# graph-embedding/node2vec

Hardware: AMD Instinct MI355X
Metric: walk-steps/sec + embedding-updates/sec on 100M-node synthetic; 1/2/4/8 GPU (higher is better)
Workload: dtype f64

## Files before the change

### node2vec_amd/csrc/n2v_walk_fast.hip

```cpp
#include "n2v_common.h"

namespace n2v {

__device__ __forceinline__ bool member_pivoted_lane(const int32_t *col, const int32_t *pivots,
                                                    int64_t first, int m, int32_t x) {
  const int64_t last = first + m;
  int64_t lo = first >> 5, hi = (last - 1) >> 5;
  while (lo < hi) {
    const int64_t mid = (lo + hi) >> 1;
    if (pivots[mid] < x)
      lo = mid + 1;
    else
      hi = mid;
  }
  int64_t a = max(first, lo << 5);
  const int64_t end = min(last, (lo << 5) + 32);
  int64_t b = end;
  while (a < b) {
    const int64_t mid = (a + b) >> 1;
    if (col[mid] < x)
      a = mid + 1;
    else
      b = mid;
  }
  return a < end && col[a] == x;
}

__global__ void pivots_build_kernel(const int32_t *__restrict__ col, int64_t n_edges,
                                    int32_t *__restrict__ pivots) {
  const int64_t n_blocks = (n_edges + 31) >> 5;
  for (int64_t j = (int64_t)blockIdx.x * blockDim.x + threadIdx.x; j < n_blocks;
       j += (int64_t)gridDim.x * blockDim.x)
    pivots[j] = col[min(32 * j + 31, n_edges - 1)];
}

__device__ __forceinline__ int lower_bound_lane(const int32_t *a, int m, int32_t x) {
  int lo = 0, hi = m;
  while (lo < hi) {
    const int mid = (lo + hi) >> 1;
    if (a[mid] < x)
      lo = mid + 1;
    else
      hi = mid;
  }
  return lo;
}

template <bool kUnit, bool kHops, bool kClassFirst, bool kSlots = false>
__global__ __launch_bounds__(256, 6) void walk_fast_kernel(
    n2v_graph g, const int32_t *__restrict__ start_ids, int64_t n_start, int32_t num_walks,
    int32_t walk_length, double p, double q, uint64_t seed, int32_t *__restrict__ walks_out,
    uint8_t *__restrict__ valid_out, uint32_t *__restrict__ status,
    unsigned long long *__restrict__ trials_out) {
  const int64_t total = n_start * (int64_t)num_walks;
  const int64_t n_lanes = (int64_t)gridDim.x * blockDim.x;
  const int L1 = walk_length + 1;
  const double inv_p = 1.0 / p, inv_q = 1.0 / q;
  const double b_lo = fmin(1.0, inv_q), b_hi = fmax(1.0, inv_q);
  const double beta_max = fmax(b_hi, inv_p);
  const bool biased = !(p == 1.0 && q == 1.0);
  const bool have_ec = kUnit && (kHops || g.edge_classes != nullptr);
  const bool have_w = have_ec && g.wedge_off != nullptr && g.wedge_pos != nullptr;
  const bool slots_tab = kSlots && have_w && g.wedge_wide != 1 && g.wedge_slots != nullptr;
  const bool inl_tab = kHops && (g.reserved2 & N2V_HOPS_INLINE_RPOS) != 0;
  int rpos_inl = -1;
  int64_t e_prev = 0;
  const bool fold_return = have_ec && inv_p > b_hi;
  const bool base_aligned = (reinterpret_cast<uintptr_t>(walks_out) & 63u) == 0;

  int64_t r = (int64_t)blockIdx.x * blockDim.x + threadIdx.x;
  bool live = false;
  int32_t s = -1, v = 0;
  int step = 0;
  uint32_t trial = 0;
  int64_t vb = 0, sb = 0, w0 = 0;
  int n = 0, m = 0;
  uint64_t h0 = 0, hstep = 0;
  unsigned long long trials = 0;
  double rho = -1.0;
  int shared = -1;
  int n_ret = 0;
  int cls = -1;
  double m_l1 = 0.0, m_l12 = 0.0, m_tot = 0.0;
  int c1 = 4, c3 = 1;
  double w1 = 0.0, d2 = 0.0, d3 = 0.0;
  if (kClassFirst) {
    double wc[3] = {inv_p, 1.0, inv_q};
    int bc[3] = {1, 2, 4};
    for (int a = 0; a < 2; ++a)
      for (int b = 0; b < 2 - a; ++b)
        if (wc[b] > wc[b + 1]) {
          const double tw = wc[b]; wc[b] = wc[b + 1]; wc[b + 1] = tw;
          const int tb = bc[b]; bc[b] = bc[b + 1]; bc[b + 1] = tb;
        }
    c1 = bc[0];
    c3 = bc[2];
    w1 = wc[0];
    d2 = wc[1] - wc[0];
    d3 = wc[2] - wc[1];
  }

  __shared__ int32_t path_tile[16][256];
  const int tid = threadIdx.x;
  int lo = 0;
  auto put = [&](int64_t a, int32_t x) { path_tile[(int)(a & 15)][tid] = x; };
  auto flush = [&](int64_t a) {
    const int k = (int)(a & 15);
    int32_t *sec = walks_out + (a & ~(int64_t)15);
    if (lo == 0 && k == 15 && base_aligned) {
#pragma unroll
      for (int u = 0; u < 4; ++u)
        reinterpret_cast<int4 *>(sec)[u] =
            make_int4(path_tile[4 * u][tid], path_tile[4 * u + 1][tid], path_tile[4 * u + 2][tid],
                      path_tile[4 * u + 3][tid]);
    } else {
      for (int kk = lo; kk <= k; ++kk) sec[kk] = path_tile[kk][tid];
    }
    lo = 0;
  };
  auto emit = [&](int pos, int32_t x) {
    const int64_t a = w0 + pos;
    put(a, x);
    if ((a & 15) == 15 || pos == walk_length) flush(a);
  };

  auto begin_walker = [&]() -> bool {
    while (r < total) {
      const int32_t start = start_ids[r / num_walks];
      const int32_t ordinal = (int32_t)(r % num_walks) + 1;
      w0 = r * (int64_t)L1;
      lo = (int)(w0 & 15);
      bool ok = true;
      if (start < 0 || (int64_t)start >= g.n_vertices) {
        atomicOr(status, N2V_ST_RANGE);
        ok = false;
      }
      if (ok) {
        vb = g.rowptr[start];
        n = (int)(g.rowptr[start + 1] - vb);
        ok = n > 0;
      }
      if (!ok || walk_length == 0) {
        emit(0, ok ? start : -1);
        for (int t = 1; t < L1; ++t) emit(t, -1);
        valid_out[r] = ok ? 1 : 0;
        r += n_lanes;
        continue;
      }
      s = -1;
      v = start;
      step = 0;
      trial = 0;
      rho = -1.0;
      shared = -1;
      cls = -1;
      emit(0, start);
      h0 = walker_stream(seed, (uint64_t)start * (uint64_t)num_walks + (uint64_t)(ordinal - 1));
      hstep = step_bits(h0, 0);
      return true;
    }
    return false;
  };

  live = begin_walker();
  while (__ballot(live) != 0ull) {
    if (!live) continue;
    const bool plain = s < 0 || !biased;
    const uint64_t bits = plain ? hstep : trial_bits(hstep, trial);
    const uint32_t u1 = (uint32_t)(bits >> 32), u2 = (uint32_t)bits;
    int pick = pick_index(u1, n);
    const bool w_wide = wedge_row_wide(g.wedge_wide, n);
    const bool have_slots = slots_tab && !w_wide;
    uint64_t wraw = 0;
    int4 ws_a = make_int4(0, 0, 0, 0), ws_b = make_int4(0, 0, 0, 0);
    if (kClassFirst && !plain) {
      if (cls < 0) {
        const double uc = (double)u2 * (1.0 / 4294967296.0) * m_tot;
        double ul = uc, wl = w1;
        cls = 7;
        if (!(uc < m_l1)) {
          if (uc < m_l12) {
            cls = 7 & ~c1;
            ul = uc - m_l1;
            wl = d2;
          } else {
            cls = c3;
            ul = uc - m_l12;
            wl = d3;
          }
        }
        if (!(cls & 4)) {
          const int cnt_r = (cls & 1) ? n_ret : 0, cnt_m = (cls & 2) ? shared : 0;
          int kk = (int)(ul / wl);
          kk = kk < cnt_r + cnt_m ? kk : cnt_r + cnt_m - 1;
          kk = kk < 0 ? 0 : kk;
          if (rpos_inl >= 0 && cnt_m == 0) {
            pick = rpos_inl + kk;
          } else if (have_slots) {
            const int4 *slot = reinterpret_cast<const int4 *>(g.wedge_slots + e_prev * 16);
            ws_a = slot[0];
            ws_b = slot[1];
            pick = kk < cnt_r ? (int)((uint32_t)ws_a.x & 0xffffu) + kk
                              : slot_entry(ws_a, ws_b, shared, kk - cnt_r,
                                           reinterpret_cast<const uint16_t *>(g.wedge_pos));
          } else {
            wraw = g.wedge_off[e_prev];
            if (kk < cnt_r) {
              pick = (int)(wraw >> N2V_WEDGE_RPOS_SHIFT) + kk;
            } else {
              const int64_t off = (int64_t)(wraw & N2V_WEDGE_OFF_MASK) + (kk - cnt_r);
              pick = w_wide ? (int)reinterpret_cast<const uint32_t *>(g.wedge_pos)[off]
                            : (int)reinterpret_cast<const uint16_t *>(g.wedge_pos)[off];
            }
          }
// ... 74 lines not shown
      }
    }
    if (!accept) {
      ++trial;
      continue;
    }
    emit(step + 1, x);
    e_prev = e;
    s = v;
    sb = vb;
    m = n;
    v = x;
    ++step;
    trial = 0;
    cls = -1;
    const bool finished = step == walk_length;
    bool dropped = false;
    if (!finished) {
      if (kHops) {
        vb = hop_row(h);
        n = hop_deg(h);
      } else {
        vb = g.rowptr[v];
        n = (int)(g.rowptr[v + 1] - vb);
      }
      dropped = n == 0;
      hstep = step_bits(h0, (uint32_t)step);
      rho = -1.0;
      shared = -1;
      if (kClassFirst) {
        uint32_t ec = kHops ? h.classes : g.edge_classes[e];
        rpos_inl = -1;
        if (inl_tab && ec != 0xffffffffu && (ec & N2V_EC_INLINE) != 0u) {
          rpos_inl = (int)(ec & N2V_EC_SHARED_MASK);
          ec = ((ec >> N2V_EC_RETURN_SHIFT) & 0x7fu) << N2V_EC_RETURN_SHIFT;
        }
        n_ret = (int)(ec >> N2V_EC_RETURN_SHIFT);
        shared = q != 1.0 ? (int)(ec & N2V_EC_SHARED_MASK) : 0;
        const int n_oth = n - n_ret - shared;
        const int n_c1 = c1 == 1 ? n_ret : (c1 == 2 ? shared : n_oth);
        const int n_c3 = c3 == 1 ? n_ret : (c3 == 2 ? shared : n_oth);
        m_l1 = (double)n * w1;
        m_l12 = m_l1 + (double)(n - n_c1) * d2;
        m_tot = m_l12 + (double)n_c3 * d3;
      } else if (have_ec && biased && !dropped) {
        uint32_t ec = kHops ? h.classes : g.edge_classes[e];
        if (inl_tab && ec != 0xffffffffu && (ec & N2V_EC_INLINE) != 0u)
          ec = ((ec >> N2V_EC_RETURN_SHIFT) & 0x7fu) << N2V_EC_RETURN_SHIFT;
        const uint32_t fR = ec >> N2V_EC_RETURN_SHIFT, fM = ec & N2V_EC_SHARED_MASK;
        if (fM != N2V_EC_SHARED_MASK) shared = (int)fM;
        if (fold_return && fR != N2V_EC_RETURN_SAT) {
          const double wr = (double)fR * inv_p;
          rho = wr / (wr + (double)n * b_hi);
        }
      }
    }
    if (finished || dropped) {
      if (dropped)
        for (int t = step + 1; t < L1; ++t) emit(t, -1);
      valid_out[r] = finished ? 1 : 0;
      r += n_lanes;
      live = begin_walker();
    }
  }
  if (trials_out && trials) atomicAdd(trials_out, trials);
}

}

extern "C" int n2v_walk_fast_launch(const n2v_graph *g, const int32_t *start_ids,
                                    int64_t n_start, int32_t num_walks, int32_t walk_length,
                                    double p, double q, uint64_t seed, int32_t *walks_out,
                                    uint8_t *valid_out, uint32_t *status, void *stream) {
  const int64_t total = n_start * (int64_t)num_walks;
  if (total == 0) return N2V_OK;
  const bool unit = g->w == nullptr && g->w64 == nullptr;
  if (!unit && !g->slots) return N2V_EINVAL;
  const int threads = 256;
  int64_t blocks = (total + threads - 1) / threads;
  const bool hops = unit && g->hops != nullptr;
  const bool cf = unit && (hops || g->edge_classes) && g->wedge_off && g->wedge_pos &&
                  !(p == 1.0 && q == 1.0);
  const bool slots = cf && hops && q < 1.0 && g->wedge_slots && g->wedge_wide != 1;
  const void *fn = slots  ? (const void *)n2v::walk_fast_kernel<true, true, true, true>
                   : cf   ? (hops ? (const void *)n2v::walk_fast_kernel<true, true, true>
                                  : (const void *)n2v::walk_fast_kernel<true, false, true>)
                   : hops ? (const void *)n2v::walk_fast_kernel<true, true, false>
                   : unit ? (const void *)n2v::walk_fast_kernel<true, false, false>
                          : (const void *)n2v::walk_fast_kernel<false, false, false>;
  const int64_t cap = n2v::resident_blocks(fn, threads, 0);
  if (blocks > cap) blocks = cap;
  unsigned long long *trials = reinterpret_cast<unsigned long long *>(status + 2);
#define N2V_FAST_LAUNCH(U, H, C)                                                                  \
  hipLaunchKernelGGL((n2v::walk_fast_kernel<U, H, C>), dim3((unsigned)blocks), dim3(threads), 0, \
                     (hipStream_t)stream, *g, start_ids, n_start, num_walks, walk_length, p, q,  \
                     seed, walks_out, valid_out, status, trials)
  if (slots)
    hipLaunchKernelGGL((n2v::walk_fast_kernel<true, true, true, true>), dim3((unsigned)blocks),
                       dim3(threads), 0, (hipStream_t)stream, *g, start_ids, n_start, num_walks,
                       walk_length, p, q, seed, walks_out, valid_out, status, trials);
  else if (cf && hops)
    N2V_FAST_LAUNCH(true, true, true);
  else if (cf)
    N2V_FAST_LAUNCH(true, false, true);
  else if (hops)
    N2V_FAST_LAUNCH(true, true, false);
  else if (unit)
    N2V_FAST_LAUNCH(true, false, false);
  else
    N2V_FAST_LAUNCH(false, false, false);
#undef N2V_FAST_LAUNCH
  N2V_HIP_CHECK(hipGetLastError());
  return N2V_OK;
}

extern "C" int n2v_pivots_build(const int32_t *col, int64_t n_edges, int32_t *pivots_out,
                                void *stream) {
  if (n_edges < 0 || (n_edges > 0 && (!col || !pivots_out))) return N2V_EINVAL;
  if (n_edges == 0) return N2V_OK;
  const int64_t n_blocks = (n_edges + 31) >> 5;
  int64_t blocks = (n_blocks + 255) / 256;
  const int64_t cap = n2v::resident_blocks((const void *)n2v::pivots_build_kernel, 256, 0) * 2;
  if (blocks > cap) blocks = cap;
  hipLaunchKernelGGL(n2v::pivots_build_kernel, dim3((unsigned)blocks), dim3(256), 0,
                     (hipStream_t)stream, col, n_edges, pivots_out);
  N2V_HIP_CHECK(hipGetLastError());
  return N2V_OK;
}
```

### node2vec_amd/csrc/n2v_walk_uniform.hip

```cpp
#include "n2v_common.h"

namespace n2v {

__device__ __forceinline__ void rank_row(const n2v_graph &g, const uint32_t *first, const uint32_t *off,
                                         uint32_t x, int64_t &vb, int &n) {
  if (x < (uint32_t)g.rank_head_n) {
    const uint64_t e = g.rank_head[x];
    vb = (int64_t)(e & N2V_HOP_ROW_MASK);
    n = (int)(e >> N2V_HOP_DEG_SHIFT);
    return;
  }
  int c = 0;
  for (int half = g.rank_classes >> 1; half > 0; half >>= 1)
    if (first[c + half] <= x) c += half;
  const uint32_t f0 = first[c], o0 = off[c];
  const uint32_t d = (off[c + 1] - o0) / (first[c + 1] - f0);
  n = (int)d;
  vb = (int64_t)(o0 + (x - f0) * d);
}

constexpr int kChunkMaxL1 = 256;

template <bool kChunked>
struct path_writer;

template <>
struct path_writer<true> {
  int32_t *at;
  int cnt;
  __device__ __forceinline__ path_writer(int32_t *walks_out, int64_t base, int64_t total, int L1, int lane,
                                         int64_t)
      : at(walks_out + base * (int64_t)L1 + lane), cnt((int)(total - base < 64 ? total - base : 64)) {}
  __device__ __forceinline__ void put(int pos, int32_t x, int) { at[pos * cnt] = x; }
};

template <>
struct path_writer<false> {
  int32_t *walks_out;
  int64_t w0;
  int lo;
  bool base_aligned;
  int32_t buf[16];
  __device__ __forceinline__ path_writer(int32_t *out, int64_t, int64_t, int L1, int, int64_t r)
      : walks_out(out), w0(r * (int64_t)L1), lo((int)((r * (int64_t)L1) & 15)),
        base_aligned((reinterpret_cast<uintptr_t>(out) & 63u) == 0) {
#pragma unroll
    for (int k = 0; k < 16; ++k) buf[k] = -1;
  }
  __device__ __forceinline__ void put(int pos, int32_t x, int walk_length) {
    const int64_t a = w0 + pos;
    const int k = (int)(a & 15);
#pragma unroll
    for (int kk = 0; kk < 16; ++kk) buf[kk] = (k == kk) ? x : buf[kk];
    if (k != 15 && pos != walk_length) return;
    int32_t *sec = walks_out + (a & ~(int64_t)15);
    if (lo == 0 && k == 15 && base_aligned) {
#pragma unroll
      for (int u = 0; u < 4; ++u)
        reinterpret_cast<int4 *>(sec)[u] =
            make_int4(buf[4 * u], buf[4 * u + 1], buf[4 * u + 2], buf[4 * u + 3]);
    } else {
#pragma unroll
      for (int kk = 0; kk < 16; ++kk)
        if (kk >= lo && kk <= k) sec[kk] = buf[kk];
    }
    lo = 0;
  }
};

template <int kHops, int kThreads, bool kChunked>
__global__ __launch_bounds__(kThreads, 8) void walk_uniform_kernel(
    n2v_graph g, const int32_t *__restrict__ start_ids, int64_t n_start, int32_t num_walks,
    int32_t walk_length, uint64_t seed, int32_t *__restrict__ walks_out,
    uint8_t *__restrict__ valid_out, uint32_t *__restrict__ status) {
  const int lane = threadIdx.x & 63;
  const int64_t total = n_start * (int64_t)num_walks;
  const int L1 = walk_length + 1;
  extern __shared__ uint32_t rank_lds[];
  const uint32_t *cls_first = rank_lds;
  const uint32_t *cls_where = rank_lds + (kHops >= 3 ? g.rank_classes : 0);
  if (kHops >= 3) {
    for (int c = threadIdx.x; c < g.rank_classes; c += kThreads) {
      rank_lds[c] = g.rank_class_first[c];
      rank_lds[g.rank_classes + c] = g.rank_class_off[c];
    }
    __syncthreads();
  }
  const bool emit_rank = kHops == 3 && g.rank_emit != 0;
  for (;;) {
    uint32_t t = 0;
    if (lane == 0) t = atomicAdd(&status[1], 64u);
    const int64_t base = (int64_t)(uint32_t)__builtin_amdgcn_readfirstlane((int)t);
    if (base >= total) break;
    const int64_t r = base + lane;
    const bool have = r < total;
    int32_t v = -1;
    uint64_t h0 = 0;
    bool alive = have;
    if (have) {
      v = start_ids[r / num_walks];
      const int32_t ordinal = (int32_t)(r % num_walks) + 1;
      h0 = walker_stream(seed, (uint64_t)v * (uint64_t)num_walks + (uint64_t)(ordinal - 1));
      if (v < 0 || (int64_t)v >= g.n_vertices) {
        atomicOr(status, N2V_ST_RANGE);
        alive = false;
      }
    }
    int64_t vb = 0;
    int n = 0;
    int32_t v_emit = v;
    if (kHops >= 3) {
      if (alive) {
        const int32_t rk = g.rank_of[v];
        if (emit_rank) v_emit = rk;
        rank_row(g, cls_first, cls_where, (uint32_t)rk, vb, n);
        alive = n > 0;
      }
    } else if (alive) {
      vb = g.rowptr[v];
      n = (int)(g.rowptr[v + 1] - vb);
      alive = n > 0;
      if (kHops == 2 && g.hop8_rowptr) vb = g.hop8_rowptr[v];
    }
    bool walking = alive;
    auto emit = path_writer<kChunked>(walks_out, base, total, L1, lane, r);
    if (have) emit.put(0, alive ? v_emit : -1, walk_length);
    for (int step = 0; step < walk_length; ++step) {
      if (ballot64(have) == 0ull) break;
      int32_t x = -1;
      if (walking) {
        const uint64_t bits = step_bits(h0, (uint32_t)step);
        const int pick = pick_index((uint32_t)(bits >> 32), n);
        if (kHops == 4) {
          const uint64_t e = reinterpret_cast<const uint64_t *>(g.rank_hops)[vb + pick];
          x = (int32_t)(uint32_t)e;
          if (step + 1 < walk_length) rank_row(g, cls_first, cls_where, (uint32_t)(e >> 32), vb, n);
        } else if (kHops == 3) {
          const uint32_t xr = g.rank_hops[vb + pick];
          x = emit_rank ? (int32_t)xr : g.rank_vertex[xr];
          if (step + 1 < walk_length) rank_row(g, cls_first, cls_where, xr, vb, n);
        } else if (kHops == 2) {
          const uint64_t h = g.hops8[vb + pick];
          const int cb = g.hop8_col_bits, rb = g.hop8_row_bits;
          x = (int32_t)(h & ((1ull << cb) - 1ull));
          vb = (int64_t)(((h >> cb) & ((1ull << rb) - 1ull)) << g.hop8_align_shift);
          const uint64_t code = h >> (cb + rb), esc = (1ull << (64 - cb - rb)) - 1ull;
          n = (int)code;
          if (code == esc) n = (int)(g.rowptr[x + 1] - g.rowptr[x]);
        } else if (kHops == 1) {
          const n2v_hop h = load_hop(g.hops + vb + pick);
          x = h.col;
          vb = hop_row(h);
          n = hop_deg(h);
        } else {
          x = g.col[vb + pick];
          if (step + 1 < walk_length) {
            vb = g.rowptr[x];
            n = (int)(g.rowptr[x + 1] - vb);
          }
        }
        if (step + 1 < walk_length && n == 0) {
          walking = false;
          alive = false;
        }
      }
      if (have) emit.put(step + 1, x, walk_length);
    }
    if (have) valid_out[r] = alive ? 1 : 0;
  }
}

constexpr int kTransposeThreads = 256, kTransposeBatch = 8;

template <int kThreads, int kBatch>
__global__ __launch_bounds__(kThreads) void walk_chunk_transpose_kernel(int32_t *__restrict__ walks,
                                                                        int64_t total, int32_t L1) {
  extern __shared__ int32_t tile[];
  const int m = L1 | 1;
  const int row0 = (int)threadIdx.x / L1, pos0 = (int)threadIdx.x % L1;
  const int drow = kThreads / L1, dpos = kThreads % L1;
  int32_t x[kBatch];
  for (int64_t base = (int64_t)blockIdx.x * 64; base < total; base += (int64_t)gridDim.x * 64) {
    const int cnt = (int)(total - base < 64 ? total - base : 64);
    int32_t *region = walks + base * (int64_t)L1;
    const int n = cnt * L1;
    const bool full = cnt == 64;
    for (int i0 = threadIdx.x; i0 < n; i0 += kThreads * kBatch) {
#pragma unroll
      for (int u = 0; u < kBatch; ++u) {
        const int i = i0 + u * kThreads;
        x[u] = i < n ? region[i] : 0;
      }
#pragma unroll
      for (int u = 0; u < kBatch; ++u) {
        const int i = i0 + u * kThreads;
        const int pos = i >> 6, l = i & 63;
        if (i < n) tile[full ? (pos << 6) + ((l * m + pos) & 63) : i] = x[u];
      }
    }
    __syncthreads();
    int row = row0, pos = pos0;
    for (int i0 = threadIdx.x; i0 < n; i0 += kThreads * kBatch) {
#pragma unroll
      for (int u = 0; u < kBatch; ++u) {
        x[u] = i0 + u * kThreads < n ? tile[pos * cnt + (full ? ((row * m + pos) & 63) : row)] : 0;
        row += drow;
        pos += dpos;
        if (pos >= L1) {
          pos -= L1;
          ++row;
        }
      }
#pragma unroll
      for (int u = 0; u < kBatch; ++u) {
        const int i = i0 + u * kThreads;
        if (i < n) region[i] = x[u];
      }
    }
    __syncthreads();
  }
}

template <int kHops, int kThreads, bool kChunked>
static hipError_t launch_walk_uniform(const n2v_graph *g, const int32_t *start_ids, int64_t n_start,
                                      int32_t num_walks, int32_t walk_length, uint64_t seed, int32_t *walks_out,
                                      uint8_t *valid_out, uint32_t *status, size_t lds, hipStream_t stream) {
  const auto fn = walk_uniform_kernel<kHops, kThreads, kChunked>;
  int64_t blocks = (n_start * (int64_t)num_walks + kThreads - 1) / kThreads;
  const int64_t cap = resident_blocks((const void *)fn, kThreads, lds);
  if (blocks > cap) blocks = cap;
  hipLaunchKernelGGL(fn, dim3((unsigned)blocks), dim3(kThreads), lds, stream, *g, start_ids, n_start, num_walks,
                     walk_length, seed, walks_out, valid_out, status);
  return hipGetLastError();
}

}

extern "C" int n2v_walk_uniform_try(const n2v_graph *g, const int32_t *start_ids, int64_t n_start,
                                    int32_t num_walks, int32_t walk_length, double p, double q,
                                    uint64_t seed, int32_t *walks_out, uint8_t *valid_out,
                                    uint32_t *status, void *stream) {
  if (g->w != nullptr || g->w64 != nullptr || p != 1.0 || q != 1.0) return 0;
  const int64_t total = n_start * (int64_t)num_walks;
  if (total >= 0xffffff00ll) return 0;
  if (total == 0) return 1;
  const int form = g->rank_hops ? (g->rank_emit == 2 ? 4 : 3) : g->hops8 ? 2 : (g->hops ? 1 : 0);
  if (form >= 3) {
    const int P = g->rank_classes;
    if (P < 2 || P > 8192 || (P & (P - 1)) || !g->rank_of || !g->rank_class_first || !g->rank_class_off ||
        g->n_edges >= (1ll << 32) ||
        g->rank_head_n < 0 || g->rank_head_n > (1 << 22) || (g->rank_head_n > 0 && !g->rank_head) ||
        (g->rank_emit == 0 && !g->rank_vertex) || g->rank_emit < 0 || g->rank_emit > 2)
      return N2V_EINVAL;
  }
  if (form == 2 && (g->hop8_col_bits < 1 || g->hop8_row_bits < 1 ||
                    g->hop8_col_bits + g->hop8_row_bits > 62 || g->hop8_align_shift < 0 ||
                    g->hop8_align_shift > 6 || (g->hop8_align_shift > 0 && !g->hop8_rowptr)))
    return N2V_EINVAL;
  if (hipMemsetAsync(status + 1, 0, sizeof(uint32_t), (hipStream_t)stream) != hipSuccess)
    return N2V_ELAUNCH;
  const hipStream_t s = (hipStream_t)stream;
  const size_t lds = form >= 3 ? (size_t)g->rank_classes * 8 : 0;
  const bool chunked = walk_length + 1 <= n2v::kChunkMaxL1;
  hipError_t e = hipSuccess;
#define N2V_UNIFORM_LAUNCH(F, T)                                                                             \
  e = chunked ? n2v::launch_walk_uniform<F, T, true>(g, start_ids, n_start, num_walks, walk_length, seed,    \
                                                     walks_out, valid_out, status, lds, s)                   \
              : n2v::launch_walk_uniform<F, T, false>(g, start_ids, n_start, num_walks, walk_length, seed,   \
                                                      walks_out, valid_out, status, lds, s)
  if (form == 4)
    N2V_UNIFORM_LAUNCH(4, 1024);
  else if (form == 3)
    N2V_UNIFORM_LAUNCH(3, 1024);
  else if (form == 2)
    N2V_UNIFORM_LAUNCH(2, 256);
  else if (form == 1)
    N2V_UNIFORM_LAUNCH(1, 256);
  else
    N2V_UNIFORM_LAUNCH(0, 256);
#undef N2V_UNIFORM_LAUNCH
  if (e != hipSuccess) return N2V_ELAUNCH;
  if (chunked) {
    int64_t chunks = (total + 63) / 64;
    const size_t tile = (size_t)64 * (size_t)(walk_length + 1) * sizeof(int32_t);
    const int64_t cap = n2v::resident_blocks(
        (const void *)n2v::walk_chunk_transpose_kernel<n2v::kTransposeThreads, n2v::kTransposeBatch>,
        n2v::kTransposeThreads, tile);
    if (chunks > cap) chunks = cap;
    hipLaunchKernelGGL((n2v::walk_chunk_transpose_kernel<n2v::kTransposeThreads, n2v::kTransposeBatch>),
                       dim3((unsigned)chunks), dim3(n2v::kTransposeThreads),
                       tile, s, walks_out, total, walk_length + 1);
    if (hipGetLastError() != hipSuccess) return N2V_ELAUNCH;
  }
  return 1;
}
```

### node2vec_amd/csrc/n2v_walk_wedge.hip

```cpp
#include "n2v_wedge_step.h"

namespace n2v {

constexpr int kWedgeThreads = 256;
constexpr int kWedgeWaves = 6;

template <int kMode>
__global__ __launch_bounds__(kWedgeThreads, kWedgeWaves) void walk_exact_wedge_kernel(
    n2v_graph g, const int32_t *__restrict__ start_ids, int64_t n_start, int32_t num_walks,
    int32_t walk_length, double p, double q, UnitConsts K, uint64_t seed,
    int32_t *__restrict__ walks_out, uint8_t *__restrict__ valid_out,
    uint32_t *__restrict__ status) {
  __shared__ int32_t path_tile[16][kWedgeThreads];
  __shared__ uint32_t stage_all[kWedgeThreads / 64][16 * 32];
  const int tid = threadIdx.x;
  const int lane = tid & 63;
  uint32_t *stage = stage_all[tid >> 6];
  const int64_t total = n_start * (int64_t)num_walks;
  const int L1 = walk_length + 1;
  const bool biased = !(p == 1.0 && q == 1.0);
  const bool need_mem = q != 1.0;
  const bool always_pair = K.bO > 1.0;
  const bool merge_r = K.bR == K.bO;
  constexpr bool kShared = kMode == 1 || kMode == 2;
  const bool base_aligned = (reinterpret_cast<uintptr_t>(walks_out) & 63u) == 0;

  int64_t w0 = 0;
  int lo = 0;
  auto flush = [&](int64_t a) {
    const int k = (int)(a & 15);
    int32_t *sec = walks_out + (a & ~(int64_t)15);
    if (lo == 0 && k == 15 && base_aligned) {
#pragma unroll
      for (int u = 0; u < 4; ++u)
        reinterpret_cast<int4 *>(sec)[u] =
            make_int4(path_tile[4 * u][tid], path_tile[4 * u + 1][tid], path_tile[4 * u + 2][tid],
                      path_tile[4 * u + 3][tid]);
    } else {
      for (int kk = lo; kk <= k; ++kk) sec[kk] = path_tile[kk][tid];
    }
    lo = 0;
  };
  auto emit = [&](int pos, int32_t x) {
    const int64_t a = w0 + pos;
    path_tile[(int)(a & 15)][tid] = x;
    if ((a & 15) == 15 || pos == walk_length) flush(a);
  };

  for (;;) {
    uint32_t t = 0;
    if (lane == 0) t = atomicAdd(&status[1], 64u);
    const int64_t base = (int64_t)(uint32_t)__builtin_amdgcn_readfirstlane((int)t);
    if (base >= total) break;
    const int64_t r = base + lane;
    const bool have = r < total;
    int32_t start = -1;
    uint64_t h0 = 0;
    bool alive = have;
    if (have) {
      start = start_ids[r / num_walks];
      const int32_t ordinal = (int32_t)(r % num_walks) + 1;
      h0 = walker_stream(seed, (uint64_t)start * (uint64_t)num_walks + (uint64_t)(ordinal - 1));
      if (start < 0 || (int64_t)start >= g.n_vertices) {
        atomicOr(status, N2V_ST_RANGE);
        alive = false;
      }
    }
    int64_t vb = 0, e_prev = 0;
    uint32_t ec_prev = 0;
    int n = 0;
    if (alive) {
      vb = g.rowptr[start];
      n = (int)(g.rowptr[start + 1] - vb);
      alive = n > 0;
    }
    w0 = r * (int64_t)L1;
    lo = (int)(w0 & 15);
    if (have) {
      emit(0, alive ? start : -1);
      if (!alive)
        for (int tt = 1; tt < L1; ++tt) emit(tt, -1);
    }
    int32_t s = -1, v = start;
    bool walking = alive;
    for (int step = 0; step < walk_length; ++step) {
      if (ballot64(walking) == 0ull) break;
      if (!walking) continue;
      const uint64_t bits = step_bits(h0, (uint32_t)step);
      const uint32_t u1 = (uint32_t)(bits >> 32), u2 = (uint32_t)bits;
      const int pick = pick_index(u1, n);
      int idx = pick;
      const bool w_wide = wedge_row_wide(g.wedge_wide, n);
      const bool step_biased = s >= 0 && biased;
      uint32_t fR = 0, fM = 0;
      if (step_biased) {
        fR = ec_prev >> N2V_EC_RETURN_SHIFT;
        fM = ec_prev & N2V_EC_SHARED_MASK;
      }
      const bool counts_ok = step_biased && fR != N2V_EC_RETURN_SAT && fM != N2V_EC_SHARED_MASK;
      uint64_t wraw = 0;
      bool w_loaded = false;
      const bool early_ok = true;
      if (counts_ok && ((need_mem && fM > 0) || ((kMode == 2 || (early_ok && always_pair)) && (fM > 0 || fR > 0)))) {
        wraw = g.wedge_off[e_prev];
        w_loaded = true;
      }
      n2v_hop h = load_hop(g.hops + vb + pick);
      int32_t x = h.col;
      if (step_biased) {
        if (!counts_ok) {
          atomicOr(status, N2V_ST_RANGE);
        } else {
          const int nR = merge_r ? 0 : (int)fR, nM = need_mem ? (int)fM : 0, nO = n - nR - nM;
          int64_t w_off = (int64_t)(wraw & N2V_WEDGE_OFF_MASK);
          const bool isR = !merge_r && x == s;
          bool isM = false;
          int lo_pick = 0;
          if (need_mem && !isR && nM > 0)
            lo_pick = wedge_lower(g.wedge_pos, w_off, nM, pick, w_wide, isM);
          double avg;
          if constexpr (kMode == 2) {
            const double b_pick = pick3(isR, isM, K.bR, K.bM, K.bO);
            const double approx = ((double)nR * K.bR + (double)nM * K.bM + (double)nO * K.bO) / (double)n;
            const double eps = ((double)n + 8.0) * 4.5e-16;
            const double r2a = (double)u2 * (1.0 / 4294967296.0);
            if (b_pick < approx * (1.0 - eps) && r2a < (b_pick / approx) * (1.0 - 2.0 * eps)) {
              avg = approx;
            } else {
              const int rp = (int)(wraw >> N2V_WEDGE_RPOS_SHIFT);
              double sum;
              if (w_wide)
                sum = lane_row_sum<uint32_t>(n, K, nR, rp, nM,
                                             reinterpret_cast<const uint32_t *>(g.wedge_pos) + w_off);
              else
                sum = lane_row_sum<uint16_t>(n, K, nR, rp, nM,
                                             reinterpret_cast<const uint16_t *>(g.wedge_pos) + w_off);
              avg = sum / (double)n;
            }
          } else {
            const int64_t isum = (int64_t)nR * K.TR + (int64_t)nM * K.TM + (int64_t)nO * K.TO;
            avg = ((double)isum * (1.0 / 1048576.0)) / (double)n;
          }
          const double p_pick = pick3(isR, isM, K.bR, K.bM, K.bO) / avg;
          const double r2 = (double)u2 * (1.0 / 4294967296.0);
          if (!(p_pick < 1.0 && r2 < p_pick)) {
            const bool uR = K.bR < avg, uM = K.bM < avg, uO = K.bO < avg;
            const bool any_under = (nR && uR) || (nM && uM) || (nO && uO);
            const bool any_over = (nR && !uR) || (nM && !uM) || (nO && !uO);
            if (!any_under || !any_over) {
              if (!(r2 < p_pick)) idx = 0;
            } else {
              if (!w_loaded) {
                wraw = g.wedge_off[e_prev];
                w_off = (int64_t)(wraw & N2V_WEDGE_OFF_MASK);
              }
              const int w_rpos = (int)(wraw >> N2V_WEDGE_RPOS_SHIFT);
              int arr = 0;
              if (uO && !(nR && uR) && !(nM && uM)) arr = 1;
              else if (!uO && nO > 0 && (!nR || uR) && (!nM || uM)) arr = 2;
              else if (kShared && uO && nR && uR && nM && !uM) arr = 3;
// ... 216 lines not shown
            const double approx = ((double)nR * K.bR + (double)nM * K.bM + (double)nO * K.bO) / (double)n;
            const double eps = ((double)n + 8.0) * 4.5e-16;
            const double r2a = (double)u2 * (1.0 / 4294967296.0);
            if (b_pick < approx * (1.0 - eps) && r2a < (b_pick / approx) * (1.0 - 2.0 * eps)) {
              avg = approx;
            } else {
              near_idx = near_step<uint32_t>(n, pick, r2a, K, nR, w_rpos, nM, list, isR, isM, lo_pick, -1);
              avg = near_idx >= 0 ? approx : lane_row_sum<uint32_t>(n, K, nR, w_rpos, nM, list) / (double)n;
            }
          } else {
            const int64_t isum = (int64_t)nR * K.TR + (int64_t)nM * K.TM + (int64_t)nO * K.TO;
            avg = ((double)isum * (1.0 / 1048576.0)) / (double)n;
          }
          const double p_pick = pick3(isR, isM, K.bR, K.bM, K.bO) / avg;
          const double r2 = (double)u2 * (1.0 / 4294967296.0);
          if (near_idx >= 0) {
            idx = near_idx;
          } else if (!(p_pick < 1.0 && r2 < p_pick)) {
            const bool uR = K.bR < avg, uM = K.bM < avg, uO = K.bO < avg;
            const bool any_under = (nR && uR) || (nM && uM) || (nO && uO);
            const bool any_over = (nR && !uR) || (nM && !uM) || (nO && !uO);
            if (!any_under || !any_over) {
              if (!(r2 < p_pick)) idx = 0;
            } else {
              int arr = 0;
              if (uO && !(nR && uR) && !(nM && uM)) arr = 1;
              else if (!uO && nO > 0 && (!nR || uR) && (!nM || uM)) arr = 2;
              else if (kShared && uO && nR && uR && nM && !uM) arr = 3;
              else if (kShared && !uO && nO > 0 && nR && !uR && nM && uM) arr = 4;
              else if (kShared && uO && nR && !uR && nM && uM) arr = 5;
              idx = pair_listed<uint32_t, kMode>(arr, n, pick, r2, K, avg, nR, w_rpos, nM, list, isR,
                                                 isM, lo_pick, stage, lane);
            }
          }
        }
      }
      if (idx >= 0) {
        next = col[vb + idx];
        edge = vb + idx;
      }
    }
    if (have) {
      next_out[i] = next;
      if (edge_out) edge_out[i] = edge;
    }
  }
}

}

int n2v_walk_wedge_try(const n2v_graph *g, const int32_t *start_ids, int64_t n_start,
                       int32_t num_walks, int32_t walk_length, double p, double q,
                       const n2v::UnitConsts &K, uint64_t seed, int32_t *walks_out,
                       uint8_t *valid_out, uint32_t *status, void *stream) {
  if (!g->hops || !g->wedge_off || !g->wedge_pos || g->w || g->w64) return 0;
  const int64_t total = n_start * (int64_t)num_walks;
  if (total >= 0xffffff00ll) return 0;
  if (total == 0) return 1;
  const bool alone_under = K.bO <= 1.0 && K.bR >= K.bO, alone_over = K.bO >= 1.0 && K.bR <= K.bO;
  if (g->wedge_wide < 0 || g->wedge_wide > 65536) return N2V_EINVAL;
  if (g->wedge_slots && g->wedge_wide != 1 && !(g->reserved & 2) &&
      (g->wedge_wide == 0 || (g->reserved2 & N2V_SLOTS_FOLDED))) {
    n2v_graph gs = *g;
    if (K.dyadic || gs.row_sums == nullptr || !(gs.row_sums_p == p && gs.row_sums_q == q) || gs.row_sums_from < 1)
      gs.row_sums = nullptr;
    g = &gs;
    auto sk = !K.dyadic    ? n2v::walk_exact_wedge_slots_kernel<2>
              : alone_under ? n2v::walk_exact_wedge_slots_kernel<0>
              : alone_over  ? n2v::walk_exact_wedge_slots_kernel<3>
                            : n2v::walk_exact_wedge_slots_kernel<1>;
    int64_t sblocks = (total + n2v::kWedgeThreads - 1) / n2v::kWedgeThreads;
    const int64_t scap = n2v::resident_blocks((const void *)sk, n2v::kWedgeThreads, 0);
    if (sblocks > scap) sblocks = scap;
    hipLaunchKernelGGL(sk, dim3((unsigned)sblocks), dim3(n2v::kWedgeThreads), 0, (hipStream_t)stream,
                       *g, start_ids, n_start, num_walks, walk_length, q, K, seed, walks_out,
                       valid_out, status);
    if (hipGetLastError() != hipSuccess) return N2V_ELAUNCH;
    return 1;
  }
  if (g->reserved2 & N2V_HOPS_INLINE_RPOS) return N2V_EINVAL;
  n2v_graph gp = *g;
  gp.row_sums = nullptr;
  g = &gp;
  auto kernel = !K.dyadic    ? n2v::walk_exact_wedge_kernel<2>
                : alone_under ? n2v::walk_exact_wedge_kernel<0>
                : alone_over  ? n2v::walk_exact_wedge_kernel<3>
                              : n2v::walk_exact_wedge_kernel<1>;
  int64_t blocks = (total + n2v::kWedgeThreads - 1) / n2v::kWedgeThreads;
  const int64_t cap = n2v::resident_blocks((const void *)kernel, n2v::kWedgeThreads, 0);
  if (blocks > cap) blocks = cap;
  hipLaunchKernelGGL(kernel, dim3((unsigned)blocks), dim3(n2v::kWedgeThreads), 0,
                     (hipStream_t)stream, *g, start_ids, n_start, num_walks, walk_length, p, q, K, seed,
                     walks_out, valid_out, status);
  if (hipGetLastError() != hipSuccess) return N2V_ELAUNCH;
  return 1;
}

int n2v_partition_step_wedge_launch(const int64_t *rowptr, const int32_t *col, int64_t lo,
                                    int64_t n_local, const int64_t *head, int32_t head_cols,
                                    const int64_t *src_ptr, const int32_t *src_ids, int32_t src_at,
                                    int64_t k, double p, double q, const n2v::UnitConsts &K, uint64_t seed,
                                    int32_t *next_out, int64_t *edge_out, uint32_t *status,
                                    void *stream) {
  const bool biased = !(p == 1.0 && q == 1.0);
  if (biased && (head_cols < 5 || !src_ptr || !src_ids)) return N2V_EINVAL;
  const bool alone_under = K.bO <= 1.0 && K.bR >= K.bO, alone_over = K.bO >= 1.0 && K.bR <= K.bO;
  auto kernel = !K.dyadic    ? n2v::partition_step_wedge_kernel<2>
                : alone_under ? n2v::partition_step_wedge_kernel<0>
                : alone_over  ? n2v::partition_step_wedge_kernel<3>
                              : n2v::partition_step_wedge_kernel<1>;
  int64_t blocks = (k + n2v::kWedgeThreads - 1) / n2v::kWedgeThreads;
  const int64_t cap = n2v::resident_blocks((const void *)kernel, n2v::kWedgeThreads, 0);
  if (blocks > cap) blocks = cap;
  hipLaunchKernelGGL(kernel, dim3((unsigned)blocks), dim3(n2v::kWedgeThreads), 0, (hipStream_t)stream,
                     rowptr, col, lo, n_local, head, (int)head_cols, src_ptr, src_ids, (int)src_at, k, p, q, K,
                     seed, next_out, edge_out, status);
  if (hipGetLastError() != hipSuccess) return N2V_ELAUNCH;
  return 1;
}

namespace n2v {
__global__ __launch_bounds__(256) void edge_row_sums_kernel(n2v_graph g, UnitConsts K, bool merge_r, bool need_mem,
                                                            const int64_t *__restrict__ edges, int64_t k,
                                                            double *__restrict__ out) {
  for (int64_t i = (int64_t)blockIdx.x * 256 + threadIdx.x; i < k; i += (int64_t)gridDim.x * 256) {
    const int64_t e = edges[i];
    if (e < 0 || e >= g.n_edges) continue;
    const int64_t x = g.col[e];
    const int64_t nn = g.rowptr[x + 1] - g.rowptr[x];
    const uint32_t ec = g.edge_classes[e];
    const uint32_t fR = ec >> N2V_EC_RETURN_SHIFT, fM = ec & N2V_EC_SHARED_MASK;
    if (fR == N2V_EC_RETURN_SAT || fM == N2V_EC_SHARED_MASK || nn <= 0 || nn >= (1 << 24)) {
      out[e] = 0.0;
      continue;
    }
    const int n = (int)nn;
    const int nR = merge_r ? 0 : (int)fR, nM = need_mem ? (int)fM : 0;
    const uint64_t wraw = g.wedge_off[e];
    const int64_t off = (int64_t)(wraw & N2V_WEDGE_OFF_MASK);
    const int rp = (int)(wraw >> N2V_WEDGE_RPOS_SHIFT);
    double sum;
    if (wedge_row_wide(g.wedge_wide, n))
      sum = lane_row_sum<uint32_t>(n, K, nR, rp, nM, reinterpret_cast<const uint32_t *>(g.wedge_pos) + off);
    else
      sum = lane_row_sum<uint16_t>(n, K, nR, rp, nM, reinterpret_cast<const uint16_t *>(g.wedge_pos) + off);
    out[e] = sum;
  }
}
}

int n2v_edge_row_sums_launch(const n2v_graph *g, const n2v::UnitConsts &K, double q, const int64_t *edges, int64_t k,
                             double *sums_out, void *stream) {
  int64_t blocks = (k + 255) / 256;
  const int64_t cap = 4 * n2v::resident_blocks((const void *)n2v::edge_row_sums_kernel, 256, 0);
  if (blocks > cap) blocks = cap;
  hipLaunchKernelGGL(n2v::edge_row_sums_kernel, dim3((unsigned)blocks), dim3(256), 0, (hipStream_t)stream, *g, K,
                     K.bR == K.bO, q != 1.0, edges, k, sums_out);
  if (hipGetLastError() != hipSuccess) return N2V_ELAUNCH;
  return N2V_OK;
}
```

Baseline: 48.43 billion.

## Extend chunked walk-major path stores plus transpose pass to fast and wedge walkers

Moves the chunked path writer and the chunk transpose kernel into a shared header and applies them to the fast (class-first) and exact wedge walk kernels when the walk length fits. Walkers in a 64-walk chunk write position-major, so each step's stores from a wavefront land in one contiguous segment. A follow-up shared-memory transpose kernel then restores the row-major walk layout. The aim is coalesced output writes from the random-walk kernels, paid for with an extra read and write pass over the walk buffer.

```diff
diff --git a/node2vec_amd/csrc/n2v_path_store.h b/node2vec_amd/csrc/n2v_path_store.h
--- /dev/null
+++ b/node2vec_amd/csrc/n2v_path_store.h
@@ -0,0 +1,118 @@
+#pragma once
+#include "n2v_common.h"
+
+namespace n2v {
+
+constexpr int kChunkMaxL1 = 256;
+
+template <bool kChunked>
+struct path_writer;
+
+template <>
+struct path_writer<true> {
+  int32_t *at;
+  int cnt;
+  path_writer() = default;
+  __device__ __forceinline__ path_writer(int32_t *walks_out, int64_t base, int64_t total, int L1, int lane,
+                                         int64_t)
+      : at(walks_out + base * (int64_t)L1 + lane), cnt((int)(total - base < 64 ? total - base : 64)) {}
+  __device__ __forceinline__ void put(int pos, int32_t x, int) { at[pos * cnt] = x; }
+};
+
+template <>
+struct path_writer<false> {
+  int32_t *walks_out;
+  int64_t w0;
+  int lo;
+  bool base_aligned;
+  int32_t buf[16];
+  __device__ __forceinline__ path_writer(int32_t *out, int64_t, int64_t, int L1, int, int64_t r)
+      : walks_out(out), w0(r * (int64_t)L1), lo((int)((r * (int64_t)L1) & 15)),
+        base_aligned((reinterpret_cast<uintptr_t>(out) & 63u) == 0) {
+#pragma unroll
+    for (int k = 0; k < 16; ++k) buf[k] = -1;
+  }
+  __device__ __forceinline__ void put(int pos, int32_t x, int walk_length) {
+    const int64_t a = w0 + pos;
+    const int k = (int)(a & 15);
+#pragma unroll
+    for (int kk = 0; kk < 16; ++kk) buf[kk] = (k == kk) ? x : buf[kk];
+    if (k != 15 && pos != walk_length) return;
+    int32_t *sec = walks_out + (a & ~(int64_t)15);
+    if (lo == 0 && k == 15 && base_aligned) {
+#pragma unroll
+      for (int u = 0; u < 4; ++u)
+        reinterpret_cast<int4 *>(sec)[u] =
+            make_int4(buf[4 * u], buf[4 * u + 1], buf[4 * u + 2], buf[4 * u + 3]);
+    } else {
+#pragma unroll
+      for (int kk = 0; kk < 16; ++kk)
+        if (kk >= lo && kk <= k) sec[kk] = buf[kk];
+    }
+    lo = 0;
+  }
+};
+
+constexpr int kTransposeThreads = 256, kTransposeBatch = 8;
+
+template <int kThreads, int kBatch>
+__global__ __launch_bounds__(kThreads) void walk_chunk_transpose_kernel(int32_t *__restrict__ walks,
+                                                                        int64_t total, int32_t L1) {
+  extern __shared__ int32_t tile[];
+  const int m = L1 | 1;
+  const int row0 = (int)threadIdx.x / L1, pos0 = (int)threadIdx.x % L1;
+  const int drow = kThreads / L1, dpos = kThreads % L1;
+  int32_t x[kBatch];
+  for (int64_t base = (int64_t)blockIdx.x * 64; base < total; base += (int64_t)gridDim.x * 64) {
+    const int cnt = (int)(total - base < 64 ? total - base : 64);
+    int32_t *region = walks + base * (int64_t)L1;
+    const int n = cnt * L1;
+    const bool full = cnt == 64;
+    for (int i0 = threadIdx.x; i0 < n; i0 += kThreads * kBatch) {
+#pragma unroll
+      for (int u = 0; u < kBatch; ++u) {
+        const int i = i0 + u * kThreads;
+        x[u] = i < n ? region[i] : 0;
+      }
+#pragma unroll
+      for (int u = 0; u < kBatch; ++u) {
+        const int i = i0 + u * kThreads;
+        const int pos = i >> 6, l = i & 63;
+        if (i < n) tile[full ? (pos << 6) + ((l * m + pos) & 63) : i] = x[u];
+      }
+    }
+    __syncthreads();
+    int row = row0, pos = pos0;
+    for (int i0 = threadIdx.x; i0 < n; i0 += kThreads * kBatch) {
+#pragma unroll
+      for (int u = 0; u < kBatch; ++u) {
+        x[u] = i0 + u * kThreads < n ? tile[pos * cnt + (full ? ((row * m + pos) & 63) : row)] : 0;
+        row += drow;
+        pos += dpos;
+        if (pos >= L1) {
+          pos -= L1;
+          ++row;
+        }
+      }
+#pragma unroll
+      for (int u = 0; u < kBatch; ++u) {
+        const int i = i0 + u * kThreads;
+        if (i < n) region[i] = x[u];
+      }
+    }
+    __syncthreads();
+  }
+}
+
+inline hipError_t chunk_transpose_launch(int32_t *walks_out, int64_t total, int32_t L1, hipStream_t stream) {
+  int64_t chunks = (total + 63) / 64;
+  const size_t tile = (size_t)64 * (size_t)L1 * sizeof(int32_t);
+  const int64_t cap = resident_blocks(
+      (const void *)walk_chunk_transpose_kernel<kTransposeThreads, kTransposeBatch>, kTransposeThreads, tile);
+  if (chunks > cap) chunks = cap;
+  hipLaunchKernelGGL((walk_chunk_transpose_kernel<kTransposeThreads, kTransposeBatch>), dim3((unsigned)chunks),
+                     dim3(kTransposeThreads), tile, stream, walks_out, total, L1);
+  return hipGetLastError();
+}
+
+}
diff --git a/node2vec_amd/csrc/n2v_walk_fast.hip b/node2vec_amd/csrc/n2v_walk_fast.hip
--- a/node2vec_amd/csrc/n2v_walk_fast.hip
+++ b/node2vec_amd/csrc/n2v_walk_fast.hip
@@ -1,4 +1,4 @@
-#include "n2v_common.h"
+#include "n2v_path_store.h"
 
 namespace n2v {
 
@@ -46,7 +46,7 @@
   return lo;
 }
 
-template <bool kUnit, bool kHops, bool kClassFirst, bool kSlots = false>
+template <bool kChunked, bool kUnit, bool kHops, bool kClassFirst, bool kSlots = false>
 __global__ __launch_bounds__(256, 6) void walk_fast_kernel(
     n2v_graph g, const int32_t *__restrict__ start_ids, int64_t n_start, int32_t num_walks,
     int32_t walk_length, double p, double q, uint64_t seed, int32_t *__restrict__ walks_out,
@@ -101,6 +101,7 @@
   }
 
   __shared__ int32_t path_tile[16][256];
+  path_writer<true> region;
   const int tid = threadIdx.x;
   int lo = 0;
   auto put = [&](int64_t a, int32_t x) { path_tile[(int)(a & 15)][tid] = x; };
@@ -119,9 +120,13 @@
     lo = 0;
   };
   auto emit = [&](int pos, int32_t x) {
-    const int64_t a = w0 + pos;
-    put(a, x);
-    if ((a & 15) == 15 || pos == walk_length) flush(a);
+    if constexpr (kChunked) {
+      region.put(pos, x, walk_length);
+    } else {
+      const int64_t a = w0 + pos;
+      put(a, x);
+      if ((a & 15) == 15 || pos == walk_length) flush(a);
+    }
   };
 
   auto begin_walker = [&]() -> bool {
@@ -130,6 +135,7 @@
       const int32_t ordinal = (int32_t)(r % num_walks) + 1;
       w0 = r * (int64_t)L1;
       lo = (int)(w0 & 15);
+      if constexpr (kChunked) region = path_writer<true>(walks_out, r & ~(int64_t)63, total, L1, (int)(r & 63), r);
       bool ok = true;
       if (start < 0 || (int64_t)start >= g.n_vertices) {
         atomicOr(status, N2V_ST_RANGE);
@@ -370,35 +376,35 @@
   const bool cf = unit && (hops || g->edge_classes) && g->wedge_off && g->wedge_pos &&
                   !(p == 1.0 && q == 1.0);
   const bool slots = cf && hops && q < 1.0 && g->wedge_slots && g->wedge_wide != 1;
-  const void *fn = slots  ? (const void *)n2v::walk_fast_kernel<true, true, true, true>
-                   : cf   ? (hops ? (const void *)n2v::walk_fast_kernel<true, true, true>
-                                  : (const void *)n2v::walk_fast_kernel<true, false, true>)
-                   : hops ? (const void *)n2v::walk_fast_kernel<true, true, false>
-                   : unit ? (const void *)n2v::walk_fast_kernel<true, false, false>
-                          : (const void *)n2v::walk_fast_kernel<false, false, false>;
-  const int64_t cap = n2v::resident_blocks(fn, threads, 0);
-  if (blocks > cap) blocks = cap;
+  const bool chunked = walk_length + 1 <= n2v::kChunkMaxL1 && cf && !slots && q >= 1.0 && p <= q;
   unsigned long long *trials = reinterpret_cast<unsigned long long *>(status + 2);
-#define N2V_FAST_LAUNCH(U, H, C)                                                                  \
-  hipLaunchKernelGGL((n2v::walk_fast_kernel<U, H, C>), dim3((unsigned)blocks), dim3(threads), 0, \
-                     (hipStream_t)stream, *g, start_ids, n_start, num_walks, walk_length, p, q,  \
-                     seed, walks_out, valid_out, status, trials)
+#define N2V_FAST_LAUNCH_AS(CH, U, H, C, S)                                                                   \
+  do {                                                                                                       \
+    const auto fn = n2v::walk_fast_kernel<CH, U, H, C, S>;                                                   \
+    const int64_t cap = n2v::resident_blocks((const void *)fn, threads, 0);                                  \
+    if (blocks > cap) blocks = cap;                                                                          \
+    hipLaunchKernelGGL(fn, dim3((unsigned)blocks), dim3(threads), 0, (hipStream_t)stream, *g, start_ids,     \
+                       n_start, num_walks, walk_length, p, q, seed, walks_out, valid_out, status, trials);   \
+  } while (0)
   if (slots)
-    hipLaunchKernelGGL((n2v::walk_fast_kernel<true, true, true, true>), dim3((unsigned)blocks),
-                       dim3(threads), 0, (hipStream_t)stream, *g, start_ids, n_start, num_walks,
-                       walk_length, p, q, seed, walks_out, valid_out, status, trials);
+    N2V_FAST_LAUNCH_AS(false, true, true, true, true);
+  else if (cf && hops && chunked)
+    N2V_FAST_LAUNCH_AS(true, true, true, true, false);
   else if (cf && hops)
-    N2V_FAST_LAUNCH(true, true, true);
+    N2V_FAST_LAUNCH_AS(false, true, true, true, false);
+  else if (cf && chunked)
+    N2V_FAST_LAUNCH_AS(true, true, false, true, false);
   else if (cf)
-    N2V_FAST_LAUNCH(true, false, true);
+    N2V_FAST_LAUNCH_AS(false, true, false, true, false);
   else if (hops)
-    N2V_FAST_LAUNCH(true, true, false);
+    N2V_FAST_LAUNCH_AS(false, true, true, false, false);
   else if (unit)
-    N2V_FAST_LAUNCH(true, false, false);
+    N2V_FAST_LAUNCH_AS(false, true, false, false, false);
   else
-    N2V_FAST_LAUNCH(false, false, false);
-#undef N2V_FAST_LAUNCH
+    N2V_FAST_LAUNCH_AS(false, false, false, false, false);
+#undef N2V_FAST_LAUNCH_AS
   N2V_HIP_CHECK(hipGetLastError());
+  if (chunked) N2V_HIP_CHECK(n2v::chunk_transpose_launch(walks_out, total, walk_length + 1, (hipStream_t)stream));
   return N2V_OK;
 }
 
diff --git a/node2vec_amd/csrc/n2v_walk_uniform.hip b/node2vec_amd/csrc/n2v_walk_uniform.hip
--- a/node2vec_amd/csrc/n2v_walk_uniform.hip
+++ b/node2vec_amd/csrc/n2v_walk_uniform.hip
@@ -1,4 +1,4 @@
-#include "n2v_common.h"
+#include "n2v_path_store.h"
 
 namespace n2v {
 
@@ -18,55 +18,6 @@
   n = (int)d;
   vb = (int64_t)(o0 + (x - f0) * d);
 }
-
-constexpr int kChunkMaxL1 = 256;
-
-template <bool kChunked>
-struct path_writer;
-
-template <>
-struct path_writer<true> {
-  int32_t *at;
-  int cnt;
-  __device__ __forceinline__ path_writer(int32_t *walks_out, int64_t base, int64_t total, int L1, int lane,
-                                         int64_t)
-      : at(walks_out + base * (int64_t)L1 + lane), cnt((int)(total - base < 64 ? total - base : 64)) {}
-  __device__ __forceinline__ void put(int pos, int32_t x, int) { at[pos * cnt] = x; }
-};
-
-template <>
-struct path_writer<false> {
-  int32_t *walks_out;
-  int64_t w0;
-  int lo;
-  bool base_aligned;
-  int32_t buf[16];
-  __device__ __forceinline__ path_writer(int32_t *out, int64_t, int64_t, int L1, int, int64_t r)
-      : walks_out(out), w0(r * (int64_t)L1), lo((int)((r * (int64_t)L1) & 15)),
-        base_aligned((reinterpret_cast<uintptr_t>(out) & 63u) == 0) {
-#pragma unroll
-    for (int k = 0; k < 16; ++k) buf[k] = -1;
-  }
-  __device__ __forceinline__ void put(int pos, int32_t x, int walk_length) {
-    const int64_t a = w0 + pos;
-    const int k = (int)(a & 15);
-#pragma unroll
-    for (int kk = 0; kk < 16; ++kk) buf[kk] = (k == kk) ? x : buf[kk];
-    if (k != 15 && pos != walk_length) return;
-    int32_t *sec = walks_out + (a & ~(int64_t)15);
-    if (lo == 0 && k == 15 && base_aligned) {
-#pragma unroll
-      for (int u = 0; u < 4; ++u)
-        reinterpret_cast<int4 *>(sec)[u] =
-            make_int4(buf[4 * u], buf[4 * u + 1], buf[4 * u + 2], buf[4 * u + 3]);
-    } else {
-#pragma unroll
-      for (int kk = 0; kk < 16; ++kk)
-        if (kk >= lo && kk <= k) sec[kk] = buf[kk];
-    }
-    lo = 0;
-  }
-};
 
 template <int kHops, int kThreads, bool kChunked>
 __global__ __launch_bounds__(kThreads, 8) void walk_uniform_kernel(
@@ -170,57 +121,6 @@
   }
 }
 
-constexpr int kTransposeThreads = 256, kTransposeBatch = 8;
-
-template <int kThreads, int kBatch>
-__global__ __launch_bounds__(kThreads) void walk_chunk_transpose_kernel(int32_t *__restrict__ walks,
-                                                                        int64_t total, int32_t L1) {
-  extern __shared__ int32_t tile[];
-  const int m = L1 | 1;
-  const int row0 = (int)threadIdx.x / L1, pos0 = (int)threadIdx.x % L1;
-  const int drow = kThreads / L1, dpos = kThreads % L1;
-  int32_t x[kBatch];
-  for (int64_t base = (int64_t)blockIdx.x * 64; base < total; base += (int64_t)gridDim.x * 64) {
-    const int cnt = (int)(total - base < 64 ? total - base : 64);
-    int32_t *region = walks + base * (int64_t)L1;
-    const int n = cnt * L1;
-    const bool full = cnt == 64;
-    for (int i0 = threadIdx.x; i0 < n; i0 += kThreads * kBatch) {
-#pragma unroll
-      for (int u = 0; u < kBatch; ++u) {
-        const int i = i0 + u * kThreads;
-        x[u] = i < n ? region[i] : 0;
-      }
-#pragma unroll
-      for (int u = 0; u < kBatch; ++u) {
-        const int i = i0 + u * kThreads;
-        const int pos = i >> 6, l = i & 63;
-        if (i < n) tile[full ? (pos << 6) + ((l * m + pos) & 63) : i] = x[u];
-      }
-    }
-    __syncthreads();
-    int row = row0, pos = pos0;
-    for (int i0 = threadIdx.x; i0 < n; i0 += kThreads * kBatch) {
-#pragma unroll
-      for (int u = 0; u < kBatch; ++u) {
-        x[u] = i0 + u * kThreads < n ? tile[pos * cnt + (full ? ((row * m + pos) & 63) : row)] : 0;
-        row += drow;
-        pos += dpos;
-        if (pos >= L1) {
-          pos -= L1;
-          ++row;
-        }
-      }
-#pragma unroll
-      for (int u = 0; u < kBatch; ++u) {
-        const int i = i0 + u * kThreads;
-        if (i < n) region[i] = x[u];
-      }
-    }
-    __syncthreads();
-  }
-}
-
 template <int kHops, int kThreads, bool kChunked>
 static hipError_t launch_walk_uniform(const n2v_graph *g, const int32_t *start_ids, int64_t n_start,
                                       int32_t num_walks, int32_t walk_length, uint64_t seed, int32_t *walks_out,
@@ -280,17 +180,7 @@
     N2V_UNIFORM_LAUNCH(0, 256);
 #undef N2V_UNIFORM_LAUNCH
   if (e != hipSuccess) return N2V_ELAUNCH;
-  if (chunked) {
-    int64_t chunks = (total + 63) / 64;
-    const size_t tile = (size_t)64 * (size_t)(walk_length + 1) * sizeof(int32_t);
-    const int64_t cap = n2v::resident_blocks(
-        (const void *)n2v::walk_chunk_transpose_kernel<n2v::kTransposeThreads, n2v::kTransposeBatch>,
-        n2v::kTransposeThreads, tile);
-    if (chunks > cap) chunks = cap;
-    hipLaunchKernelGGL((n2v::walk_chunk_transpose_kernel<n2v::kTransposeThreads, n2v::kTransposeBatch>),
-                       dim3((unsigned)chunks), dim3(n2v::kTransposeThreads),
-                       tile, s, walks_out, total, walk_length + 1);
-    if (hipGetLastError() != hipSuccess) return N2V_ELAUNCH;
-  }
+  if (chunked && n2v::chunk_transpose_launch(walks_out, total, walk_length + 1, s) != hipSuccess)
+    return N2V_ELAUNCH;
   return 1;
 }
diff --git a/node2vec_amd/csrc/n2v_walk_wedge.hip b/node2vec_amd/csrc/n2v_walk_wedge.hip
--- a/node2vec_amd/csrc/n2v_walk_wedge.hip
+++ b/node2vec_amd/csrc/n2v_walk_wedge.hip
@@ -1,3 +1,4 @@
+#include "n2v_path_store.h"
 #include "n2v_wedge_step.h"
 
 namespace n2v {
@@ -5,7 +6,7 @@
 constexpr int kWedgeThreads = 256;
 constexpr int kWedgeWaves = 6;
 
-template <int kMode>
+template <int kMode, bool kChunked>
 __global__ __launch_bounds__(kWedgeThreads, kWedgeWaves) void walk_exact_wedge_kernel(
     n2v_graph g, const int32_t *__restrict__ start_ids, int64_t n_start, int32_t num_walks,
     int32_t walk_length, double p, double q, UnitConsts K, uint64_t seed,
@@ -41,10 +42,15 @@
     }
     lo = 0;
   };
+  path_writer<true> region;
   auto emit = [&](int pos, int32_t x) {
-    const int64_t a = w0 + pos;
-    path_tile[(int)(a & 15)][tid] = x;
-    if ((a & 15) == 15 || pos == walk_length) flush(a);
+    if constexpr (kChunked) {
+      region.put(pos, x, walk_length);
+    } else {
+      const int64_t a = w0 + pos;
+      path_tile[(int)(a & 15)][tid] = x;
+      if ((a & 15) == 15 || pos == walk_length) flush(a);
+    }
   };
 
   for (;;) {
@@ -76,6 +82,7 @@
     }
     w0 = r * (int64_t)L1;
     lo = (int)(w0 & 15);
+    if constexpr (kChunked) region = path_writer<true>(walks_out, base, total, L1, lane, r);
     if (have) {
       emit(0, alive ? start : -1);
       if (!alive)
@@ -458,10 +465,14 @@
   n2v_graph gp = *g;
   gp.row_sums = nullptr;
   g = &gp;
-  auto kernel = !K.dyadic    ? n2v::walk_exact_wedge_kernel<2>
-                : alone_under ? n2v::walk_exact_wedge_kernel<0>
-                : alone_over  ? n2v::walk_exact_wedge_kernel<3>
-                              : n2v::walk_exact_wedge_kernel<1>;
+  const bool chunked = walk_length + 1 <= n2v::kChunkMaxL1;
+#define N2V_WEDGE_INSTANCE(CHUNKED)                             \
+  (!K.dyadic     ? n2v::walk_exact_wedge_kernel<2, CHUNKED>     \
+   : alone_under ? n2v::walk_exact_wedge_kernel<0, CHUNKED>     \
+   : alone_over  ? n2v::walk_exact_wedge_kernel<3, CHUNKED>     \
+                 : n2v::walk_exact_wedge_kernel<1, CHUNKED>)
+  auto kernel = chunked ? N2V_WEDGE_INSTANCE(true) : N2V_WEDGE_INSTANCE(false);
+#undef N2V_WEDGE_INSTANCE
   int64_t blocks = (total + n2v::kWedgeThreads - 1) / n2v::kWedgeThreads;
   const int64_t cap = n2v::resident_blocks((const void *)kernel, n2v::kWedgeThreads, 0);
   if (blocks > cap) blocks = cap;
@@ -469,6 +480,8 @@
                      (hipStream_t)stream, *g, start_ids, n_start, num_walks, walk_length, p, q, K, seed,
                      walks_out, valid_out, status);
   if (hipGetLastError() != hipSuccess) return N2V_ELAUNCH;
+  if (chunked && n2v::chunk_transpose_launch(walks_out, total, walk_length + 1, (hipStream_t)stream) != hipSuccess)
+    return N2V_ELAUNCH;
   return 1;
 }
 
```

Result: no change. 47.98 billion (median of 2 runs) (-0.9%).
